# huawei-noah/Speech-Backbones

Measured on AMD Instinct MI355X. Metric: mel-frames/sec at N=50 reverse-diffusion, 80x1024 batch, higher is better.
Workload: dtype f32 storage, f16 hi*hi MFMA + fp8 cross-term MFMA (3x3 Block convolutions, Upsample; bf16x3 elsewhere), f32 accumulate; 1 GPU; BASELINE config 2: Grad-TTS LJSpeech decoder, N=50, B=16/GPU synthetic 80x1024 mels, all-ones mask; per_gpu_batch=16, frames=1024, parallelism=utterance-shard x1, weights=seed-0 default init, Rezero.g=0.02, output_finite=True, conv_kernel=conv_ws.hip (persistent, wave-specialised), sub_batch_streams=0, hip_graph=False, launches_per_euler_step=64

## Files before the change

speech-backbones_amd/csrc/attn.hip:

```cpp
#include <cstring>
#include "common.h"
#include "kernels.h"

#ifndef GTTS_ATTN_HPW
#define GTTS_ATTN_HPW 2
#endif

namespace gtts {

struct AttnCtxArgs {
    const void *x;
    const unsigned char *wkv;
    float *partials;
    int C, HW, nstage, tiles, tps, nrec, nsplit, B;
    AttnTail tail;
};

__device__ __forceinline__ void pack8_split(const float (&v)[8], u32x4 &hi, u32x4 &lo) {
    bf16x8 vh, vl;
#pragma unroll
    for (int i = 0; i < 8; ++i) {
        __bf16 h, l;
        split_bf16(v[i], h, l);
        vh[i] = h;
        vl[i] = l;
    }
    hi = *reinterpret_cast<u32x4 *>(&vh);
    lo = *reinterpret_cast<u32x4 *>(&vl);
}

template <int NSPLIT, int FULLC, typename AT = float, int HPW = 1, int TAIL = 0>
__global__ __launch_bounds__(256 * HPW, HPW == 1 ? 2 : 1) void attn_ctx_kernel(const AttnCtxArgs a) {
    constexpr int AB = (int)sizeof(AT);
    static_assert(!TAIL || (FULLC && AB == 4), "the fused tail: whole 32-channel stages, fp32 storage");
    constexpr int KCH = ATTN_KCH, NKG = 2 * KCH;
    constexpr int NKGT = NKG / HPW;
    constexpr int WHEAD = 2 * NKG * 64;
    static_assert(HPW == 1 || HPW == 2, "one or two heads per workgroup");
    constexpr int SM16 = 2 * NKG * 256 + HPW * WHEAD;
    static_assert((size_t)SM16 * 16 >= (size_t)4 * HPW * ATTN_REC * 4, "merge records must fit the staging buffer");
    __shared__ __attribute__((aligned(16))) u32x4 s_all[SM16];
    u32x4 *s_ah = s_all, *s_al = s_all + NKG * 256;
    u32x4 *s_wall = s_all + 2 * NKG * 256;

    const int tid = threadIdx.x, lane = tid & 63;
    const int t255 = tid & 255, hw = __builtin_amdgcn_readfirstlane(tid >> 8);
    const int wave = (tid >> 6) & 3;
    const int l31 = lane & 31, kgl = lane >> 5;
    constexpr int HG = 4 / HPW;
    const int nsl = gridDim.x / (HG * a.B);
    const int wg = xcd_slot(blockIdx.x, gridDim.x);
    const int head = (wg % HG) * HPW + hw, slice = (wg / HG) % nsl, b = (wg / HG) / nsl;
    u32x4 *s_w = s_wall + hw * WHEAD;
    const int tile0 = slice * a.tps;
    const int tile1 = min(tile0 + a.tps, a.tiles);
    const AT *xb = reinterpret_cast<const AT *>(a.x) + (size_t)b * a.C * a.HW;
    const u32x4 *wblk = reinterpret_cast<const u32x4 *>(a.wkv) + (size_t)head * a.nstage * (2 * NKG * 64);

    float raw[NKGT][8];
    u32x4 wregs[KCH];
    const unsigned long long xaddr = reinterpret_cast<unsigned long long>(xb);
    const unsigned xlo = __builtin_amdgcn_readfirstlane((unsigned)xaddr);
    const unsigned xhi = __builtin_amdgcn_readfirstlane((unsigned)(xaddr >> 32));
    const int xbytes = a.C * a.HW * AB;
    const __amdgpu_buffer_rsrc_t rsx = __builtin_amdgcn_make_buffer_rsrc(
        reinterpret_cast<void *>(((unsigned long long)xhi << 32) | xlo), 0, __builtin_amdgcn_readfirstlane(xbytes), 0x00020000);
    [[maybe_unused]] float rawh[NKGT][8], tmask = 0.f;
    [[maybe_unused]] __amdgpu_buffer_rsrc_t rsh = rsx, rsi = rsx;
    [[maybe_unused]] const bool tail_store = (wg % HG) == 0;
    if constexpr (TAIL) {
        auto mk = [&](const void *p) {
            const unsigned long long u = reinterpret_cast<unsigned long long>(reinterpret_cast<const AT *>(p) + (size_t)b * a.C * a.HW);
            const unsigned lo = __builtin_amdgcn_readfirstlane((unsigned)u), hi = __builtin_amdgcn_readfirstlane((unsigned)(u >> 32));
            return __builtin_amdgcn_make_buffer_rsrc(reinterpret_cast<void *>(((unsigned long long)hi << 32) | lo), 0,
                                                     __builtin_amdgcn_readfirstlane(xbytes), 0x00020000);
        };
        rsh = mk(a.tail.h);
        rsi = mk(a.tail.xin);
    }
    auto apply_tail = [&](int tile, int stage) {
        if constexpr (TAIL) {
            const int n = tile * 256 + t255;
            const int voff = n < a.HW ? n * AB : xbytes;
#pragma unroll
            for (int kg = 0; kg < NKGT; ++kg) {
                const int cb = stage * 16 * KCH + (hw * NKGT + kg) * 8;
#pragma unroll
                for (int i = 0; i < 8; ++i) {
                    const float sc = a.tail.esc[(size_t)b * a.C + cb + i], sh = a.tail.esh[(size_t)b * a.C + cb + i];
                    const float v = tail_value(rawh[kg][i], raw[kg][i], sc, sh, tmask);
                    raw[kg][i] = v;
                    if (tail_store) __builtin_amdgcn_raw_buffer_store_b32(__builtin_bit_cast(int, v), rsx, voff, (cb + i) * a.HW * 4, GTTS_OUT_NT);
                }
            }
        }
    };
    auto load = [&](int tile, int stage) {
        const int n = tile * 256 + t255;
        const int voff = n < a.HW ? n * AB : xbytes;
        if constexpr (TAIL) {
            if (stage == 0) tmask = n < a.HW ? a.tail.mask[(size_t)b * a.tail.T + ((size_t)(n % a.tail.W) << a.tail.lvl)] : 0.f;
        }
#pragma unroll
        for (int kg = 0; kg < NKGT; ++kg) {
            const int cb = stage * 16 * KCH + (hw * NKGT + kg) * 8;
#pragma unroll
            for (int i = 0; i < 8; ++i) {
                const int c = FULLC ? cb + i : min(cb + i, a.C - 1);
                float v;
                if constexpr (TAIL) {
                    v = __builtin_bit_cast(float, __builtin_amdgcn_raw_buffer_load_b32(rsi, voff, c * a.HW * 4, 0));
                    rawh[kg][i] = __builtin_bit_cast(float, __builtin_amdgcn_raw_buffer_load_b32(rsh, voff, c * a.HW * 4, 0));
                } else if constexpr (AB == 4) v = __builtin_bit_cast(float, __builtin_amdgcn_raw_buffer_load_b32(rsx, voff, c * a.HW * 4, 0));
                else v = __builtin_bit_cast(float, (unsigned)(unsigned short)__builtin_amdgcn_raw_buffer_load_b16(rsx, voff, c * a.HW * 2, 0) << 16);
                raw[kg][i] = (FULLC || cb + i < a.C) ? v : 0.f;
            }
        }
        const u32x4 *g = wblk + (size_t)stage * (2 * NKG * 64);
#pragma unroll
        for (int j = 0; j < KCH; ++j) wregs[j] = g[t255 + j * 256];
    };

    const float NEG_INF = -__builtin_inff();
    float m_run = NEG_INF, z_run = 0.f;
    f32x16 ctx;
#pragma unroll
    for (int r = 0; r < 16; ++r) ctx[r] = 0.f;
    constexpr bool lo_on = NSPLIT > 1;

    load(tile0, 0);
    for (int tile = tile0; tile < tile1; ++tile) {
        f32x16 acc[2][2];
#pragma unroll
        for (int pf = 0; pf < 2; ++pf)
#pragma unroll
            for (int cf = 0; cf < 2; ++cf)
#pragma unroll
                for (int r = 0; r < 16; ++r) acc[pf][cf][r] = 0.f;

        for (int stage = 0; stage < a.nstage; ++stage) {
            apply_tail(tile, stage);
            lds_barrier();
#pragma unroll
            for (int kg = 0; kg < NKGT; ++kg) {
                u32x4 hi, lo;
                pack8_split(raw[kg], hi, lo);
                s_ah[(hw * NKGT + kg) * 256 + t255] = hi;
                s_al[(hw * NKGT + kg) * 256 + t255] = lo;
            }
#pragma unroll
            for (int j = 0; j < KCH; ++j) s_w[t255 + j * 256] = wregs[j];
            lds_barrier();
            if (stage + 1 < a.nstage) load(tile, stage + 1);
            else if (tile + 1 < tile1) load(tile + 1, 0);
#pragma unroll
            for (int kc = 0; kc < KCH; ++kc) {
                bf16x8 xh[2], xl[2], wh[2], wl[2];
#pragma unroll
                for (int pf = 0; pf < 2; ++pf) {
                    const int xi = (kc * 2 + kgl) * 256 + wave * 64 + pf * 32 + l31;
                    xh[pf] = *reinterpret_cast<const bf16x8 *>(&s_ah[xi]);
                    xl[pf] = *reinterpret_cast<const bf16x8 *>(&s_al[xi]);
                }
#pragma unroll
                for (int cf = 0; cf < 2; ++cf) {
                    const int wi = (kc * 2 + kgl) * 64 + cf * 32 + l31;
                    wh[cf] = *reinterpret_cast<const bf16x8 *>(&s_w[wi]);
                    wl[cf] = *reinterpret_cast<const bf16x8 *>(&s_w[wi + NKG * 64]);
                }
#pragma unroll
                for (int pf = 0; pf < 2; ++pf)
#pragma unroll
                    for (int cf = 0; cf < 2; ++cf) {
                        if (lo_on) {
                            acc[pf][cf] = __builtin_amdgcn_mfma_f32_32x32x16_bf16(xl[pf], wh[cf], acc[pf][cf], 0, 0, 0);
                            acc[pf][cf] = __builtin_amdgcn_mfma_f32_32x32x16_bf16(xh[pf], wl[cf], acc[pf][cf], 0, 0, 0);
                        }
                        acc[pf][cf] = __builtin_amdgcn_mfma_f32_32x32x16_bf16(xh[pf], wh[cf], acc[pf][cf], 0, 0, 0);
                    }
            }
        }

        const int nbase = tile * 256 + wave * 64 + 4 * kgl;
        const bool full = tile * 256 + 256 <= a.HW;
        float tmax = NEG_INF;
        if (full) {
#pragma unroll
            for (int pf = 0; pf < 2; ++pf)
#pragma unroll
                for (int rg = 0; rg < 16; ++rg) tmax = fmaxf(tmax, acc[pf][0][rg]);
        } else {
#pragma unroll
            for (int pf = 0; pf < 2; ++pf)
#pragma unroll
                for (int rg = 0; rg < 16; ++rg) {
                    const int n = nbase + pf * 32 + (rg & 3) + 8 * (rg >> 2);
                    if (n < a.HW) tmax = fmaxf(tmax, acc[pf][0][rg]);
                }
        }
        tmax = fmaxf(tmax, __shfl_xor(tmax, 32, 64));
        const float m_new = fmaxf(m_run, tmax);
        const float alpha = (m_run == NEG_INF) ? 0.f : __expf(m_run - m_new);
        const float msub = (m_new == NEG_INF) ? 0.f : m_new;
        constexpr float LOG2E = 1.44269504088896340736f;
        float psum = 0.f;
        if (full) {
#pragma unroll
            for (int pf = 0; pf < 2; ++pf)
#pragma unroll
                for (int rg = 0; rg < 16; ++rg) {
                    const float p = __builtin_amdgcn_exp2f((acc[pf][0][rg] - msub) * LOG2E);
                    acc[pf][0][rg] = p;
                    psum += p;
                }
        } else {
#pragma unroll
            for (int pf = 0; pf < 2; ++pf)
#pragma unroll
                for (int rg = 0; rg < 16; ++rg) {
                    const int n = nbase + pf * 32 + (rg & 3) + 8 * (rg >> 2);
                    const float p = (n < a.HW) ? __builtin_amdgcn_exp2f((acc[pf][0][rg] - msub) * LOG2E) : 0.f;
                    acc[pf][0][rg] = p;
                    psum += p;
                }
        }
        psum += __shfl_xor(psum, 32, 64);
        z_run = z_run * alpha + psum;
        m_run = m_new;
        if (__builtin_amdgcn_ballot_w64(alpha != 1.f) != 0ull) {
#pragma unroll
            for (int rg = 0; rg < 16; ++rg) {
                const int d = (rg & 3) + 8 * (rg >> 2) + 4 * kgl;
                ctx[rg] *= __shfl(alpha, d, 64);
            }
        }
#pragma unroll
        for (int pf = 0; pf < 2; ++pf)
#pragma unroll
            for (int hh = 0; hh < 2; ++hh) {
                float pv[8], vv[8];
#pragma unroll
                for (int i = 0; i < 8; ++i) {
                    pv[i] = acc[pf][0][hh * 8 + i];
                    vv[i] = acc[pf][1][hh * 8 + i];
                }
                u32x4 ph, pl, vh, vl;
                pack8_split(pv, ph, pl);
                pack8_split(vv, vh, vl);
                const bf16x8 Ph = *reinterpret_cast<bf16x8 *>(&ph), Pl = *reinterpret_cast<bf16x8 *>(&pl);
                const bf16x8 Vh = *reinterpret_cast<bf16x8 *>(&vh), Vl = *reinterpret_cast<bf16x8 *>(&vl);
                if (lo_on) {
                    ctx = __builtin_amdgcn_mfma_f32_32x32x16_bf16(Pl, Vh, ctx, 0, 0, 0);
                    ctx = __builtin_amdgcn_mfma_f32_32x32x16_bf16(Ph, Vl, ctx, 0, 0, 0);
                }
                ctx = __builtin_amdgcn_mfma_f32_32x32x16_bf16(Ph, Vh, ctx, 0, 0, 0);
            }
    }

    __syncthreads();
    float (*s_mrg)[ATTN_REC] = reinterpret_cast<float (*)[ATTN_REC]>(s_all) + hw * 4;
    {
        float *mine = s_mrg[wave];
        if (kgl == 0) {
            mine[l31] = m_run;
            mine[32 + l31] = z_run;
        }
#pragma unroll
        for (int rg = 0; rg < 16; ++rg) {
            const int d = (rg & 3) + 8 * (rg >> 2) + 4 * kgl;
            mine[64 + d * 32 + l31] = ctx[rg];
        }
    }
    __syncthreads();
    float *rec = a.partials + ((((size_t)b * 4 + head) * a.nrec) + (size_t)slice) * ATTN_REC;
#pragma unroll
    for (int k = 0; k < 4; ++k) {
        const int idx = t255 + 256 * k, d = idx >> 5;
        float M = NEG_INF;
#pragma unroll
        for (int w = 0; w < 4; ++w) M = fmaxf(M, s_mrg[w][d]);
        float acc_c = 0.f, acc_z = 0.f;
#pragma unroll
        for (int w = 0; w < 4; ++w) {
            const float mw = s_mrg[w][d];
            const float sc = (mw == NEG_INF) ? 0.f : __expf(mw - M);
            acc_c = fmaf(s_mrg[w][64 + idx], sc, acc_c);
            acc_z = fmaf(s_mrg[w][32 + d], sc, acc_z);
        }
        rec[64 + idx] = acc_c;
        if ((idx & 31) == 0) {
            rec[d] = M;
            rec[32 + d] = acc_z;
        }
    }
}

template <int NSPLIT, typename AT, int TAIL = 0>
__global__ __launch_bounds__(256, 2) void attn_ctx64_kernel(const AttnCtxArgs a) {
    constexpr int AB = (int)sizeof(AT);
    constexpr int C = 64, NKGT = C / 8;
    constexpr bool lo_on = NSPLIT > 1;
    __shared__ __attribute__((aligned(16))) u32x4 s_ah[NKGT * 64];
    __shared__ __attribute__((aligned(16))) u32x4 s_al[NKGT * 64];
    __shared__ __attribute__((aligned(16))) u32x4 s_w[4][1024];

    const int tid = threadIdx.x, lane = tid & 63;
    const int wave = __builtin_amdgcn_readfirstlane(tid >> 6);
    const int l31 = lane & 31, kgl = lane >> 5;
    const int nsl = gridDim.x / a.B;
    const int wg = xcd_slot(blockIdx.x, gridDim.x);
    const int slice = wg % nsl, b = wg / nsl;
    const int head = wave;
    const int tile0 = slice * a.tps, tile1 = min(tile0 + a.tps, a.tiles);
    const AT *xb = reinterpret_cast<const AT *>(a.x) + (size_t)b * C * a.HW;

    {
        const u32x4 *wsrc = reinterpret_cast<const u32x4 *>(a.wkv) + (size_t)head * 1024;
        u32x4 wr[16];
#pragma unroll
        for (int i = 0; i < 16; ++i) wr[i] = wsrc[lane + 64 * i];
#pragma unroll
        for (int i = 0; i < 16; ++i) s_w[wave][lane + 64 * i] = wr[i];
    }

    const unsigned long long xaddr = reinterpret_cast<unsigned long long>(xb);
    const unsigned xlo = __builtin_amdgcn_readfirstlane((unsigned)xaddr);
    const unsigned xhi = __builtin_amdgcn_readfirstlane((unsigned)(xaddr >> 32));
    const int xbytes = C * a.HW * AB;
    const __amdgpu_buffer_rsrc_t rsx = __builtin_amdgcn_make_buffer_rsrc(
        reinterpret_cast<void *>(((unsigned long long)xhi << 32) | xlo), 0, __builtin_amdgcn_readfirstlane(xbytes), 0x00020000);
    float raw[2][8];
    [[maybe_unused]] float rawh[2][8], tsc[2][8], tsh[2][8], tmask = 0.f;
    [[maybe_unused]] __amdgpu_buffer_rsrc_t rsh = rsx, rsi = rsx;
    if constexpr (TAIL) {
        static_assert(!TAIL || AB == 4, "the fused tail is the fp32-storage form");
        auto mk = [&](const void *p) {
            const unsigned long long u = reinterpret_cast<unsigned long long>(reinterpret_cast<const AT *>(p) + (size_t)b * C * a.HW);
            const unsigned lo = __builtin_amdgcn_readfirstlane((unsigned)u), hi = __builtin_amdgcn_readfirstlane((unsigned)(u >> 32));
            return __builtin_amdgcn_make_buffer_rsrc(reinterpret_cast<void *>(((unsigned long long)hi << 32) | lo), 0,
                                                     __builtin_amdgcn_readfirstlane(xbytes), 0x00020000);
        };
        rsh = mk(a.tail.h);
        rsi = mk(a.tail.xin);
#pragma unroll
        for (int it = 0; it < 2; ++it)
#pragma unroll
            for (int i = 0; i < 8; ++i) {
                const int c = (it * 4 + wave) * 8 + i;
                tsc[it][i] = a.tail.esc[(size_t)b * C + c];
                tsh[it][i] = a.tail.esh[(size_t)b * C + c];
            }
    }
    auto load = [&](int tile) {
        const int n = tile * 64 + lane;
        const int voff = n < a.HW ? n * AB : xbytes;
#pragma unroll
        for (int it = 0; it < 2; ++it)
#pragma unroll
            for (int i = 0; i < 8; ++i) {
                const int c = (it * 4 + wave) * 8 + i;
                if constexpr (TAIL) {
                    raw[it][i] = __builtin_bit_cast(float, __builtin_amdgcn_raw_buffer_load_b32(rsi, voff, c * a.HW * 4, 0));
                    rawh[it][i] = __builtin_bit_cast(float, __builtin_amdgcn_raw_buffer_load_b32(rsh, voff, c * a.HW * 4, 0));
                } else if constexpr (AB == 4) raw[it][i] = __builtin_bit_cast(float, __builtin_amdgcn_raw_buffer_load_b32(rsx, voff, c * a.HW * 4, 0));
                else raw[it][i] = __builtin_bit_cast(float, (unsigned)(unsigned short)__builtin_amdgcn_raw_buffer_load_b16(rsx, voff, c * a.HW * 2, 0) << 16);
            }
        if constexpr (TAIL) tmask = n < a.HW ? a.tail.mask[(size_t)b * a.tail.T + ((size_t)(n % a.tail.W) << a.tail.lvl)] : 0.f;
    };
    auto apply_tail = [&](int tile) {
        if constexpr (TAIL) {
            const int n = tile * 64 + lane;
            const int voff = n < a.HW ? n * AB : xbytes;
#pragma unroll
            for (int it = 0; it < 2; ++it)
#pragma unroll
                for (int i = 0; i < 8; ++i) {
                    const int c = (it * 4 + wave) * 8 + i;
                    const float v = tail_value(rawh[it][i], raw[it][i], tsc[it][i], tsh[it][i], tmask);
                    raw[it][i] = v;
                    __builtin_amdgcn_raw_buffer_store_b32(__builtin_bit_cast(int, v), rsx, voff, c * a.HW * 4, GTTS_OUT_NT);
                }
        }
    };

    const float NEG_INF = -__builtin_inff();
    float m_run = NEG_INF, z_run = 0.f;
    f32x16 ctx;
#pragma unroll
    for (int r = 0; r < 16; ++r) ctx[r] = 0.f;

    load(tile0);
    for (int tile = tile0; tile < tile1; ++tile) {
        apply_tail(tile);
        lds_barrier();
#pragma unroll
        for (int it = 0; it < 2; ++it) {
            u32x4 hi, lo;
            pack8_split(raw[it], hi, lo);
            s_ah[(it * 4 + wave) * 64 + lane] = hi;
            if (lo_on) s_al[(it * 4 + wave) * 64 + lane] = lo;
        }
        lds_barrier();
        load(min(tile + 1, tile1 - 1));

        f32x16 acc[2][2];
#pragma unroll
        for (int pf = 0; pf < 2; ++pf)
#pragma unroll
            for (int cf = 0; cf < 2; ++cf)
#pragma unroll
                for (int r = 0; r < 16; ++r) acc[pf][cf][r] = 0.f;
#pragma unroll
        for (int s = 0; s < 4; ++s) {
            bf16x8 xh[2], xl[2], wh[2], wl[2];
#pragma unroll
            for (int pf = 0; pf < 2; ++pf) {
                const int xi = (s * 2 + kgl) * 64 + pf * 32 + l31;
                xh[pf] = *reinterpret_cast<const bf16x8 *>(&s_ah[xi]);
                if (lo_on) xl[pf] = *reinterpret_cast<const bf16x8 *>(&s_al[xi]);
            }
#pragma unroll
            for (int cf = 0; cf < 2; ++cf) {
                const int wi = (s >> 1) * 512 + ((s & 1) * 2 + kgl) * 64 + cf * 32 + l31;
                wh[cf] = *reinterpret_cast<const bf16x8 *>(&s_w[wave][wi]);
                if (lo_on) wl[cf] = *reinterpret_cast<const bf16x8 *>(&s_w[wave][wi + 256]);
            }
#pragma unroll
            for (int pf = 0; pf < 2; ++pf)
#pragma unroll
                for (int cf = 0; cf < 2; ++cf) {
                    if (lo_on) {
                        acc[pf][cf] = __builtin_amdgcn_mfma_f32_32x32x16_bf16(xl[pf], wh[cf], acc[pf][cf], 0, 0, 0);
                        acc[pf][cf] = __builtin_amdgcn_mfma_f32_32x32x16_bf16(xh[pf], wl[cf], acc[pf][cf], 0, 0, 0);
                    }
                    acc[pf][cf] = __builtin_amdgcn_mfma_f32_32x32x16_bf16(xh[pf], wh[cf], acc[pf][cf], 0, 0, 0);
                }
        }

        const int nbase = tile * 64 + 4 * kgl;
        const bool full = tile * 64 + 64 <= a.HW;
        float tmax = NEG_INF;
        if (full) {
#pragma unroll
            for (int pf = 0; pf < 2; ++pf)
#pragma unroll
                for (int rg = 0; rg < 16; ++rg) tmax = fmaxf(tmax, acc[pf][0][rg]);
        } else {
#pragma unroll
            for (int pf = 0; pf < 2; ++pf)
#pragma unroll
                for (int rg = 0; rg < 16; ++rg) {
                    const int n = nbase + pf * 32 + (rg & 3) + 8 * (rg >> 2);
                    if (n < a.HW) tmax = fmaxf(tmax, acc[pf][0][rg]);
                }
        }
        tmax = fmaxf(tmax, __shfl_xor(tmax, 32, 64));
        const float m_new = fmaxf(m_run, tmax);
        const float alpha = (m_run == NEG_INF) ? 0.f : __expf(m_run - m_new);
        const float msub = (m_new == NEG_INF) ? 0.f : m_new;
        constexpr float LOG2E = 1.44269504088896340736f;
        float psum = 0.f;
        if (full) {
#pragma unroll
            for (int pf = 0; pf < 2; ++pf)
#pragma unroll
                for (int rg = 0; rg < 16; ++rg) {
                    const float p = __builtin_amdgcn_exp2f((acc[pf][0][rg] - msub) * LOG2E);
                    acc[pf][0][rg] = p;
                    psum += p;
                }
        } else {
#pragma unroll
            for (int pf = 0; pf < 2; ++pf)
#pragma unroll
                for (int rg = 0; rg < 16; ++rg) {
                    const int n = nbase + pf * 32 + (rg & 3) + 8 * (rg >> 2);
                    const float p = (n < a.HW) ? __builtin_amdgcn_exp2f((acc[pf][0][rg] - msub) * LOG2E) : 0.f;
                    acc[pf][0][rg] = p;
                    psum += p;
                }
        }
        psum += __shfl_xor(psum, 32, 64);
        z_run = z_run * alpha + psum;
        m_run = m_new;
        if (__builtin_amdgcn_ballot_w64(alpha != 1.f) != 0ull) {
#pragma unroll
            for (int rg = 0; rg < 16; ++rg) {
                const int d = (rg & 3) + 8 * (rg >> 2) + 4 * kgl;
                ctx[rg] *= __shfl(alpha, d, 64);
            }
        }
#pragma unroll
        for (int pf = 0; pf < 2; ++pf)
#pragma unroll
            for (int hh = 0; hh < 2; ++hh) {
                float pv[8], vv[8];
#pragma unroll
                for (int i = 0; i < 8; ++i) {
                    pv[i] = acc[pf][0][hh * 8 + i];
                    vv[i] = acc[pf][1][hh * 8 + i];
                }
                u32x4 ph, pl, vh, vl;
                pack8_split(pv, ph, pl);
                pack8_split(vv, vh, vl);
                const bf16x8 Ph = *reinterpret_cast<bf16x8 *>(&ph), Pl = *reinterpret_cast<bf16x8 *>(&pl);
                const bf16x8 Vh = *reinterpret_cast<bf16x8 *>(&vh), Vl = *reinterpret_cast<bf16x8 *>(&vl);
                if (lo_on) {
                    ctx = __builtin_amdgcn_mfma_f32_32x32x16_bf16(Pl, Vh, ctx, 0, 0, 0);
                    ctx = __builtin_amdgcn_mfma_f32_32x32x16_bf16(Ph, Vl, ctx, 0, 0, 0);
                }
                ctx = __builtin_amdgcn_mfma_f32_32x32x16_bf16(Ph, Vh, ctx, 0, 0, 0);
            }
    }

    float *rec = a.partials + ((((size_t)b * 4 + head) * a.nrec) + (size_t)slice) * ATTN_REC;
    if (kgl == 0) {
        rec[l31] = m_run;
        rec[32 + l31] = z_run;
    }
#pragma unroll
    for (int rg = 0; rg < 16; ++rg) {
        const int d = (rg & 3) + 8 * (rg >> 2) + 4 * kgl;
        rec[64 + d * 32 + l31] = ctx[rg];
    }
}

template <int NSPLIT, typename AT, int TAIL>
static hipError_t launch_ctx64(const AttnCtxArgs &a, dim3 grid, hipStream_t st, std::string *name) {
    if (name) return kernel_name(name, "gtts::attn_ctx64_kernel", NSPLIT, act_name<AT>(), TAIL);
    hipLaunchKernelGGL((attn_ctx64_kernel<NSPLIT, AT, TAIL>), grid, dim3(256), 0, st, a);
    return hipGetLastError();
}
template <int NSPLIT, int FULLC, typename AT, int TAIL>
static hipError_t launch_ctx(const AttnCtxArgs &a, int nslices, hipStream_t st, std::string *name) {
    constexpr int HPW = GTTS_ATTN_HPW;
    if (name) return kernel_name(name, "gtts::attn_ctx_kernel", NSPLIT, FULLC, act_name<AT>(), HPW, TAIL);
    hipLaunchKernelGGL((attn_ctx_kernel<NSPLIT, FULLC, AT, HPW, TAIL>), dim3(nslices * (4 / HPW) * a.B), dim3(256 * HPW), 0, st, a);
    return hipGetLastError();
}

hipError_t launch_attn_ctx(const void *x, const unsigned char *wkv, float *partials, int B, int C, int HW, int nsplit,
                           hipStream_t st, int act_bf16, const AttnTail *tail, std::string *name) {
    AttnGeom g = attn_geom(HW, C);
    if ((size_t)C * HW * 4 >= ((size_t)1 << 31)) return hipErrorInvalidValue;
    if (tail != nullptr && (C % 32 != 0 || act_bf16)) return hipErrorInvalidValue;
    if (act_bf16 && nsplit > 1) return hipErrorInvalidValue;
    AttnCtxArgs a;
    memset(&a, 0, sizeof(a));
    if (tail != nullptr) a.tail = *tail;
    a.x = x; a.wkv = wkv; a.partials = partials; a.C = C; a.HW = HW;
    a.nstage = (C + 16 * ATTN_KCH - 1) / (16 * ATTN_KCH);
    a.tiles = g.tiles; a.tps = g.tps; a.nrec = g.nrec; a.nsplit = nsplit; a.B = B;
    if (attn_head_per_wave(C)) {
        static_assert(ATTN_KCH == 2, "attn_ctx64_kernel indexes the packed k|v blocks as 32-channel stages");
        const dim3 grid64(g.nslices * B);
        if (act_bf16) return launch_ctx64<1, __bf16, 0>(a, grid64, st, name);
        if (tail != nullptr) return nsplit > 1 ? launch_ctx64<2, float, 1>(a, grid64, st, name) : launch_ctx64<1, float, 1>(a, grid64, st, name);
        return nsplit > 1 ? launch_ctx64<2, float, 0>(a, grid64, st, name) : launch_ctx64<1, float, 0>(a, grid64, st, name);
    }
    if (act_bf16) return C % 32 == 0 ? launch_ctx<1, 1, __bf16, 0>(a, g.nslices, st, name) : launch_ctx<1, 0, __bf16, 0>(a, g.nslices, st, name);
    if (tail != nullptr) return nsplit > 1 ? launch_ctx<2, 1, float, 1>(a, g.nslices, st, name) : launch_ctx<1, 1, float, 1>(a, g.nslices, st, name);
    if (C % 32 == 0) return nsplit > 1 ? launch_ctx<2, 1, float, 0>(a, g.nslices, st, name) : launch_ctx<1, 1, float, 0>(a, g.nslices, st, name);
    return nsplit > 1 ? launch_ctx<2, 0, float, 0>(a, g.nslices, st, name) : launch_ctx<1, 0, float, 0>(a, g.nslices, st, name);
}

__global__ __launch_bounds__(1024) void attn_merge_kernel(const float *__restrict__ partials, float *__restrict__ ctxn,
                                                           int nrec) {
    extern __shared__ float sm[];
    float *s_w = sm;
    float *s_red = sm + (size_t)nrec * 32;
    float *s_M = s_red + 1024;
    float *s_Zi = s_M + 32;
    const int head = blockIdx.x, b = blockIdx.y, tid = threadIdx.x;
    const int d = tid & 31, g = tid >> 5;
    const float *rec = partials + ((size_t)b * 4 + head) * nrec * ATTN_REC;
    const float NEG_INF = -__builtin_inff();
    float mx = NEG_INF;
    for (int i = g; i < nrec; i += 32) mx = fmaxf(mx, rec[(size_t)i * ATTN_REC + d]);
    s_red[g * 32 + d] = mx;
    __syncthreads();
    if (g == 0) {
        float M = NEG_INF;
        for (int k = 0; k < 32; ++k) M = fmaxf(M, s_red[k * 32 + d]);
        s_M[d] = M;
    }
    __syncthreads();
    const float M = s_M[d];
    float zz = 0.f;
    for (int i = g; i < nrec; i += 32) {
        const float mi = rec[(size_t)i * ATTN_REC + d];
        const float w = (mi == NEG_INF) ? 0.f : expf(mi - M);
        s_w[i * 32 + d] = w;
        zz += rec[(size_t)i * ATTN_REC + 32 + d] * w;
    }
    __syncthreads();
    s_red[g * 32 + d] = zz;
    __syncthreads();
    if (g == 0) {
        float Z = 0.f;
        for (int k = 0; k < 32; ++k) Z += s_red[k * 32 + d];
        s_Zi[d] = 1.0f / Z;
    }
    __syncthreads();
    const int dd = tid >> 5;
    float acc = 0.f;
    const float *cp = rec + 64 + tid;
    int i = 0;
    for (; i + 4 <= nrec; i += 4) {
        const float c0 = cp[(size_t)(i + 0) * ATTN_REC], c1 = cp[(size_t)(i + 1) * ATTN_REC];
        const float c2 = cp[(size_t)(i + 2) * ATTN_REC], c3 = cp[(size_t)(i + 3) * ATTN_REC];
        acc = fmaf(c0, s_w[(i + 0) * 32 + dd], acc);
        acc = fmaf(c1, s_w[(i + 1) * 32 + dd], acc);
        acc = fmaf(c2, s_w[(i + 2) * 32 + dd], acc);
        acc = fmaf(c3, s_w[(i + 3) * 32 + dd], acc);
    }
    for (; i < nrec; ++i) acc = fmaf(cp[(size_t)i * ATTN_REC], s_w[i * 32 + dd], acc);
    ctxn[(((size_t)b * 4 + head) * 1024) + tid] = acc * s_Zi[dd];
}

hipError_t launch_attn_merge(const float *partials, float *ctxn, int B, int nrec, hipStream_t st) {
    const size_t smem = ((size_t)nrec * 32 + 1024 + 64) * sizeof(float);
    if (smem > 160 * 1024) return hipErrorInvalidValue;
    if (smem > 48 * 1024) {
        const hipError_t e = raise_dyn_lds<&attn_merge_kernel>(smem);
        if (e != hipSuccess) return e;
    }
    hipLaunchKernelGGL(attn_merge_kernel, dim3(4, B), dim3(1024), smem, st, partials, ctxn, nrec);
    return hipGetLastError();
}

constexpr int FOLD_CO = 8;
struct AttnFoldArgs {
    const float *ctxn, *wq, *wout, *bout, *g;
    unsigned char *wpk;
    size_t wpk_bstride;
    float *biasb;
    int C, MT, nkg;
    int ndn;
    const float *dn_w, *dn_wo, *dn_vw;
    unsigned char *dn_wpk;
    size_t dn_bstride;
    float *dn_btab;
    int dn_MT, dn_nkg;
};
__global__ __launch_bounds__(256) void attn_fold_kernel(const AttnFoldArgs a) {
    __shared__ float s_U[FOLD_CO][128];
    __shared__ float s_part[4][FOLD_CO][128];
    const int co0 = blockIdx.x * FOLD_CO, b = blockIdx.z, tid = threadIdx.x;
    const int C = a.C;
    const int tap = (int)blockIdx.y < a.ndn ? (int)blockIdx.y : -1;
    const float *wout = tap >= 0 ? a.dn_wo + (size_t)tap * C * 128 : a.wout;
    const float *cb = a.ctxn + (size_t)b * 4096;
    {
        const int j = tid & 127, h = j >> 5, d = j & 31;
        const float4 *cx = reinterpret_cast<const float4 *>(cb + (h * 32 + d) * 32);
        float4 cv[8];
#pragma unroll
        for (int e = 0; e < 8; ++e) cv[e] = cx[e];
#pragma unroll
        for (int rr = 0; rr < FOLD_CO / 2; ++rr) {
            const int r = (tid >> 7) * (FOLD_CO / 2) + rr;
            const float4 *wo = reinterpret_cast<const float4 *>(wout + (size_t)(co0 + r) * 128 + h * 32);
            float acc = 0.f;
#pragma unroll
            for (int e = 0; e < 8; ++e) {
                const float4 w4 = wo[e];
                acc = fmaf(w4.x, cv[e].x, acc); acc = fmaf(w4.y, cv[e].y, acc);
                acc = fmaf(w4.z, cv[e].z, acc); acc = fmaf(w4.w, cv[e].w, acc);
            }
            s_U[r][j] = acc;
        }
    }
    __syncthreads();
    const float gv = a.g[0];
    const int MT = tap >= 0 ? a.dn_MT : a.MT, nkg = tap >= 0 ? a.dn_nkg : a.nkg;
    const int ncot = (C + MT - 1) / MT;
    __bf16 *wp = tap >= 0 ? reinterpret_cast<__bf16 *>(a.dn_wpk + (size_t)b * a.dn_bstride)
                          : reinterpret_cast<__bf16 *>(a.wpk + (size_t)b * a.wpk_bstride);
    const int ky = tap >= 0 ? tap / 3 : 0, kx = tap >= 0 ? tap - 3 * ky : 0;
    const int nst = tap >= 0 ? 3 : 1, tps = nst;
    const int Cc = C < 256 ? C : 256;
    const int nj = 256 / Cc >= 4 ? 4 : (256 / Cc >= 2 ? 2 : 1);
    const int jq = tid / Cc, cl = tid - jq * Cc;
    const int jn = 128 / nj;
    const bool active = jq < nj;
    for (int ci = cl; ci < C; ci += Cc) {
        float acc[FOLD_CO];
#pragma unroll
        for (int r = 0; r < FOLD_CO; ++r) acc[r] = 0.f;
        const float *qp = a.wq + (size_t)(active ? jq * jn : 0) * C + ci;
        for (int j0 = 0; j0 < (active ? jn : 0); j0 += 8) {
            float q[8];
#pragma unroll
            for (int u = 0; u < 8; ++u) q[u] = qp[(size_t)(j0 + u) * C];
#pragma unroll
            for (int u = 0; u < 8; ++u)
#pragma unroll
                for (int r = 0; r < FOLD_CO; ++r) acc[r] = fmaf(s_U[r][jq * jn + j0 + u], q[u], acc[r]);
        }
        if (nj > 1) {
            if (active && jq > 0) {
#pragma unroll
                for (int r = 0; r < FOLD_CO; ++r) s_part[jq][r][cl] = acc[r];
            }
            __syncthreads();
            if (jq == 0) {
                for (int k = 1; k < nj; ++k)
#pragma unroll
                    for (int r = 0; r < FOLD_CO; ++r) acc[r] += s_part[k][r][cl];
            }
        }
        if (jq == 0) {
            const int chunk = ci / (8 * nkg), kg = (ci >> 3) % nkg, i = ci & 7;
#pragma unroll
            for (int r = 0; r < FOLD_CO; ++r) {
                const int co = co0 + r, cot = co / MT, m = co % MT;
                const size_t blk = ((size_t)chunk * nst + ky) * ncot + cot;
                const size_t blk_elems = (size_t)tps * MT * 16 * nkg;
                const size_t e_hi = blk * blk_elems + ((size_t)((0 * tps + kx) * nkg + kg) * MT + m) * 8 + i;
                const size_t e_lo = blk * blk_elems + ((size_t)((1 * tps + kx) * nkg + kg) * MT + m) * 8 + i;
                const float v = tap >= 0 ? fmaf(acc[r], gv, a.dn_w[((size_t)co * C + ci) * 9 + tap]) : acc[r] * gv;
                __bf16 hi, lo;
                split_bf16(v, hi, lo);
                wp[e_hi] = hi;
                wp[e_lo] = lo;
            }
        }
    }
    if (tap < 0 && tid < FOLD_CO) a.biasb[(size_t)b * C + co0 + tid] = gv * a.bout[co0 + tid];
    if (tap == 0 && tid < FOLD_CO) {
        const int co = co0 + tid;
        float *t = a.dn_btab + (size_t)b * 6 * C + co;
#pragma unroll
        for (int k = 0; k < 3; ++k) {
            const float v0 = a.dn_vw[(size_t)(0 + k) * C + co], v1 = a.dn_vw[(size_t)(3 + k) * C + co], v2 = a.dn_vw[(size_t)(6 + k) * C + co];
            t[(size_t)(0 + k) * C] = gv * (v1 + v2);
            t[(size_t)(3 + k) * C] = gv * ((v0 + v1) + v2);
        }
    }
}

hipError_t launch_attn_fold(const float *ctxn, const float *wq, const float *wout, const float *bout, const float *g,
                            unsigned char *wpk, size_t wpk_bstride, float *biasb, int B, int C, hipStream_t st,
                            const AttnFoldDn *dn) {
    if (C % 16 != 0) return hipErrorInvalidValue;
    ConvGeom geom = conv_geom(CONV_P1, C, C);
    if (C % (16 * geom.kch) != 0) return hipErrorInvalidValue;
    if (wpk == nullptr && dn == nullptr) return hipErrorInvalidValue;
    AttnFoldArgs a;
    memset(&a, 0, sizeof(a));
    a.ctxn = ctxn; a.wq = wq; a.wout = wout; a.bout = bout; a.g = g;
    a.wpk = wpk; a.wpk_bstride = wpk_bstride; a.biasb = biasb;
    a.C = C; a.MT = geom.MT; a.nkg = 2 * geom.kch;
    if (dn != nullptr) {
        ConvGeom gd = conv_geom(CONV_DN, C, C);
        if (C % (16 * gd.kch) != 0 || C % gd.MT != 0 || gd.nst != 3 || gd.tps != 3) return hipErrorInvalidValue;
        if (dn->bstride < conv_packed_bytes(CONV_DN, C, C)) return hipErrorInvalidValue;
        a.ndn = 9;
        a.dn_w = dn->w; a.dn_wo = dn->wo; a.dn_vw = dn->vw;
        a.dn_wpk = dn->wpk; a.dn_bstride = dn->bstride; a.dn_btab = dn->btab;
        a.dn_MT = gd.MT; a.dn_nkg = 2 * gd.kch;
    }
    hipLaunchKernelGGL(attn_fold_kernel, dim3(C / FOLD_CO, a.ndn + (wpk != nullptr ? 1 : 0), B), dim3(256), 0, st, a);
    return hipGetLastError();
}

__global__ __launch_bounds__(128) void attn_dn_precompose_kernel(const float *__restrict__ w, const float *__restrict__ wout,
                                                                  const float *__restrict__ bout, float *__restrict__ wo,
                                                                  float *__restrict__ vw, int C) {
    const int co = blockIdx.x, tap = blockIdx.y, j = threadIdx.x;
    const float *wr = w + (size_t)co * C * 9 + tap;
    float acc = 0.f, accb = 0.f;
    for (int c = 0; c < C; ++c) {
        const float wv = wr[(size_t)c * 9];
        acc = fmaf(wv, wout[(size_t)c * 128 + j], acc);
        accb = fmaf(wv, bout[c], accb);
    }
    wo[((size_t)tap * C + co) * 128 + j] = acc;
    if (j == 0) vw[(size_t)tap * C + co] = accb;
}

hipError_t launch_attn_dn_precompose(const float *w, const float *wout, const float *bout, float *wo, float *vw, int C, hipStream_t st) {
    hipLaunchKernelGGL(attn_dn_precompose_kernel, dim3(C, 9), dim3(128), 0, st, w, wout, bout, wo, vw, C);
    return hipGetLastError();
}

}
```

Before: 55910 mel-frames/s.

## Split attention merge across row groups and vectorize fold weight packing stores

The merge kernel now splits each head across four smaller workgroups when there are many partial records, and hoists the first two record loads into registers to cut load latency. The fold kernel is templated on the j-split factor. It prefetches q weights through buffer loads with double buffering and reads s_U as float4. It stages packed bf16 hi/lo weights in LDS so they can be written as 16-byte vector stores instead of scattered 2-byte stores. Optional memtime tracing instrumentation is added behind a debug macro, and new alignment checks reject unaligned packed-weight buffers.

```diff
diff --git a/speech-backbones_amd/csrc/attn.hip b/speech-backbones_amd/csrc/attn.hip
--- a/speech-backbones_amd/csrc/attn.hip
+++ b/speech-backbones_amd/csrc/attn.hip
@@ -564,68 +564,134 @@
     return nsplit > 1 ? launch_ctx<2, 0, float, 0>(a, g.nslices, st, name) : launch_ctx<1, 0, float, 0>(a, g.nslices, st, name);
 }
 
+#ifndef GTTS_DIAG
+#undef GTTS_GLUE_TRACE
+#endif
+#ifndef GTTS_GLUE_TRACE
+#define GTTS_GLUE_TRACE 0
+#endif
+#if GTTS_GLUE_TRACE
+constexpr int GLUE_TRACE_MERGE = 4, GLUE_TRACE_N = 8 * 16 * 16 * 9;
+__device__ unsigned long long g_glue_trace[GLUE_TRACE_N];
+extern "C" int gtts_debug_trace_glue(unsigned long long *dst, int n) {
+    return (int)hipMemcpyFromSymbol(dst, HIP_SYMBOL(g_glue_trace), sizeof(unsigned long long) * (n < GLUE_TRACE_N ? n : GLUE_TRACE_N));
+}
+__device__ __forceinline__ int merge_trace_slot(int nrec) { return nrec == 16 ? 0 : (nrec == 20 ? 1 : (nrec == 64 ? 2 : 3)); }
+__device__ __forceinline__ unsigned long long *glue_trace_row(int slot, int wg, int wave) {
+    return g_glue_trace + (((size_t)slot * 16 + wg) * 16 + wave) * 9;
+}
+#define MT_MARK(k) do { const unsigned long long tr_now = __builtin_amdgcn_s_memtime(); tr_sum[k] += tr_now - tr_t; tr_t = tr_now; } while (0)
+#else
+#define MT_MARK(k) do { } while (0)
+#endif
 __global__ __launch_bounds__(1024) void attn_merge_kernel(const float *__restrict__ partials, float *__restrict__ ctxn,
                                                            int nrec) {
     extern __shared__ float sm[];
+    const int RD = (int)blockDim.x >> 5;
+    const int R = 32 / RD;
     float *s_w = sm;
-    float *s_red = sm + (size_t)nrec * 32;
-    float *s_M = s_red + 1024;
-    float *s_Zi = s_M + 32;
-    const int head = blockIdx.x, b = blockIdx.y, tid = threadIdx.x;
-    const int d = tid & 31, g = tid >> 5;
+    float *s_red = sm + (size_t)nrec * RD;
+    float *s_M = s_red + 32 * RD;
+    float *s_Zi = s_M + RD;
+    const int head = (int)blockIdx.x / R, row0 = ((int)blockIdx.x - head * R) * RD, b = blockIdx.y, tid = threadIdx.x;
+    const int d = tid & (RD - 1), g = tid / RD;
+#if GTTS_GLUE_TRACE
+    const bool tr_on = (tid & 63) == 0;
+    unsigned long long tr_sum[8] = {0, 0, 0, 0, 0, 0, 0, 0};
+    unsigned long long tr_t = __builtin_amdgcn_s_memtime();
+    const unsigned long long tr_entry = tr_t;
+#endif
     const float *rec = partials + ((size_t)b * 4 + head) * nrec * ATTN_REC;
+    const float *recd = rec + row0 + d;
     const float NEG_INF = -__builtin_inff();
-    float mx = NEG_INF;
-    for (int i = g; i < nrec; i += 32) mx = fmaxf(mx, rec[(size_t)i * ATTN_REC + d]);
-    s_red[g * 32 + d] = mx;
+    const bool h0 = g < nrec, h1 = g + 32 < nrec;
+    const float *r0 = recd + (size_t)(h0 ? g : 0) * ATTN_REC, *r1 = recd + (size_t)(h1 ? g + 32 : 0) * ATTN_REC;
+    const float m0 = r0[0], m1 = r1[0], z0 = r0[32], z1 = r1[32];
+    float mx = fmaxf(h0 ? m0 : NEG_INF, h1 ? m1 : NEG_INF);
+    for (int i = g + 64; i < nrec; i += 32) mx = fmaxf(mx, recd[(size_t)i * ATTN_REC]);
+    MT_MARK(0);
+    s_red[g * RD + d] = mx;
     __syncthreads();
     if (g == 0) {
         float M = NEG_INF;
-        for (int k = 0; k < 32; ++k) M = fmaxf(M, s_red[k * 32 + d]);
+        for (int k = 0; k < 32; ++k) M = fmaxf(M, s_red[k * RD + d]);
         s_M[d] = M;
     }
     __syncthreads();
+    MT_MARK(1);
     const float M = s_M[d];
     float zz = 0.f;
-    for (int i = g; i < nrec; i += 32) {
-        const float mi = rec[(size_t)i * ATTN_REC + d];
+    if (h0) {
+        const float w = (m0 == NEG_INF) ? 0.f : expf(m0 - M);
+        s_w[g * RD + d] = w;
+        zz += z0 * w;
+    }
+    if (h1) {
+        const float w = (m1 == NEG_INF) ? 0.f : expf(m1 - M);
+        s_w[(g + 32) * RD + d] = w;
+        zz += z1 * w;
+    }
+    for (int i = g + 64; i < nrec; i += 32) {
+        const float mi = recd[(size_t)i * ATTN_REC];
         const float w = (mi == NEG_INF) ? 0.f : expf(mi - M);
-        s_w[i * 32 + d] = w;
-        zz += rec[(size_t)i * ATTN_REC + 32 + d] * w;
+        s_w[i * RD + d] = w;
+        zz += recd[(size_t)i * ATTN_REC + 32] * w;
     }
     __syncthreads();
-    s_red[g * 32 + d] = zz;
+    s_red[g * RD + d] = zz;
     __syncthreads();
     if (g == 0) {
         float Z = 0.f;
-        for (int k = 0; k < 32; ++k) Z += s_red[k * 32 + d];
+        for (int k = 0; k < 32; ++k) Z += s_red[k * RD + d];
         s_Zi[d] = 1.0f / Z;
     }
     __syncthreads();
+    MT_MARK(2);
     const int dd = tid >> 5;
     float acc = 0.f;
-    const float *cp = rec + 64 + tid;
+    const float *cp = rec + 64 + row0 * 32 + tid;
     int i = 0;
+    for (; i + 16 <= nrec; i += 16) {
+        float c[16];
+#pragma unroll
+        for (int u = 0; u < 16; ++u) c[u] = cp[(size_t)(i + u) * ATTN_REC];
+#pragma unroll
+        for (int u = 0; u < 16; ++u) acc = fmaf(c[u], s_w[(i + u) * RD + dd], acc);
+    }
     for (; i + 4 <= nrec; i += 4) {
         const float c0 = cp[(size_t)(i + 0) * ATTN_REC], c1 = cp[(size_t)(i + 1) * ATTN_REC];
         const float c2 = cp[(size_t)(i + 2) * ATTN_REC], c3 = cp[(size_t)(i + 3) * ATTN_REC];
-        acc = fmaf(c0, s_w[(i + 0) * 32 + dd], acc);
-        acc = fmaf(c1, s_w[(i + 1) * 32 + dd], acc);
-        acc = fmaf(c2, s_w[(i + 2) * 32 + dd], acc);
-        acc = fmaf(c3, s_w[(i + 3) * 32 + dd], acc);
-    }
-    for (; i < nrec; ++i) acc = fmaf(cp[(size_t)i * ATTN_REC], s_w[i * 32 + dd], acc);
-    ctxn[(((size_t)b * 4 + head) * 1024) + tid] = acc * s_Zi[dd];
-}
+        acc = fmaf(c0, s_w[(i + 0) * RD + dd], acc);
+        acc = fmaf(c1, s_w[(i + 1) * RD + dd], acc);
+        acc = fmaf(c2, s_w[(i + 2) * RD + dd], acc);
+        acc = fmaf(c3, s_w[(i + 3) * RD + dd], acc);
+    }
+    for (; i < nrec; ++i) acc = fmaf(cp[(size_t)i * ATTN_REC], s_w[i * RD + dd], acc);
+    MT_MARK(3);
+    ctxn[(((size_t)b * 4 + head) * 1024) + row0 * 32 + tid] = acc * s_Zi[dd];
+#if GTTS_GLUE_TRACE
+    if (tr_on && blockIdx.y == 0 && blockIdx.x < 16) {
+        __builtin_amdgcn_s_waitcnt(0);
+        MT_MARK(4);
+        unsigned long long *t = glue_trace_row(GLUE_TRACE_MERGE + merge_trace_slot(nrec), blockIdx.x, tid >> 6);
+        for (int q = 0; q < 8; ++q) t[q] = tr_sum[q];
+        t[8] = tr_t - tr_entry;
+    }
+#endif
+}
+
+static inline int attn_merge_row_groups(int nrec) { return nrec >= 48 ? 4 : 1; }
 
 hipError_t launch_attn_merge(const float *partials, float *ctxn, int B, int nrec, hipStream_t st) {
-    const size_t smem = ((size_t)nrec * 32 + 1024 + 64) * sizeof(float);
+    if (nrec < 1) return hipErrorInvalidValue;
+    const int R = attn_merge_row_groups(nrec);
+    const size_t smem = ((size_t)nrec * (32 / R) + 1024 / R + 2 * (32 / R)) * sizeof(float);
     if (smem > 160 * 1024) return hipErrorInvalidValue;
     if (smem > 48 * 1024) {
         const hipError_t e = raise_dyn_lds<&attn_merge_kernel>(smem);
         if (e != hipSuccess) return e;
     }
-    hipLaunchKernelGGL(attn_merge_kernel, dim3(4, B), dim3(1024), smem, st, partials, ctxn, nrec);
+    hipLaunchKernelGGL(attn_merge_kernel, dim3(4 * R, B), dim3(1024 / R), smem, st, partials, ctxn, nrec);
     return hipGetLastError();
 }
 
@@ -643,14 +709,58 @@
     float *dn_btab;
     int dn_MT, dn_nkg;
 };
-__global__ __launch_bounds__(256) void attn_fold_kernel(const AttnFoldArgs a) {
-    __shared__ float s_U[FOLD_CO][128];
-    __shared__ float s_part[4][FOLD_CO][128];
+constexpr int FOLD_QB = 32;
+template <int NJ>
+__device__ __forceinline__ void attn_fold_impl(const AttnFoldArgs &a, float (*s_U)[128], float (*s_part)[FOLD_CO][128],
+                                               __bf16 (*s_o)[FOLD_CO][256 + 8]) {
+    constexpr int JN = 128 / NJ;
+    constexpr int QB = FOLD_QB;
+    constexpr int NB = JN / QB;
     const int co0 = blockIdx.x * FOLD_CO, b = blockIdx.z, tid = threadIdx.x;
     const int C = a.C;
     const int tap = (int)blockIdx.y < a.ndn ? (int)blockIdx.y : -1;
     const float *wout = tap >= 0 ? a.dn_wo + (size_t)tap * C * 128 : a.wout;
     const float *cb = a.ctxn + (size_t)b * 4096;
+    const int Cc = C < 256 ? C : 256;
+    const int jq = tid / Cc, cl = tid - jq * Cc;
+    const bool active = jq < NJ;
+    const int jb = (active ? jq : 0) * JN;
+#if GTTS_GLUE_TRACE
+    const bool tr_on = (tid & 63) == 0;
+    unsigned long long tr_sum[8] = {0, 0, 0, 0, 0, 0, 0, 0};
+    unsigned long long tr_t = __builtin_amdgcn_s_memtime();
+    const unsigned long long tr_entry = tr_t;
+#endif
+    float q[2][QB], dw[FOLD_CO];
+#pragma unroll
+    for (int r = 0; r < FOLD_CO; ++r) dw[r] = 0.f;
+    int ci0 = 0, cis = cl;
+    auto rsrc = [](const float *p, int bytes) {
+        const unsigned long long u = reinterpret_cast<unsigned long long>(p);
+        const unsigned lo = __builtin_amdgcn_readfirstlane((unsigned)u), hi = __builtin_amdgcn_readfirstlane((unsigned)(u >> 32));
+        return __builtin_amdgcn_make_buffer_rsrc(reinterpret_cast<void *>(((unsigned long long)hi << 32) | lo), 0,
+                                                 __builtin_amdgcn_readfirstlane(bytes), 0x00020000);
+    };
+    const __amdgpu_buffer_rsrc_t rs_q = rsrc(a.wq, 128 * C * 4);
+    const __amdgpu_buffer_rsrc_t rs_w = rsrc(tap >= 0 ? a.dn_w : a.wq, tap >= 0 ? C * C * 36 : 128 * C * 4);
+    auto load_q = [&](float (&dst)[QB], int kb) {
+        const int voff = (jb * C + cis) * 4;
+#pragma unroll
+        for (int u = 0; u < QB; ++u)
+            dst[u] = __builtin_bit_cast(float, __builtin_amdgcn_raw_buffer_load_b32(rs_q, voff, (kb * QB + u) * C * 4, 0));
+    };
+    auto preload = [&]() {
+        load_q(q[0], 0);
+        if (NB > 1) load_q(q[1], 1);
+        if (tap >= 0 && jq == 0) {
+#pragma unroll
+            for (int r = 0; r < FOLD_CO; ++r)
+                dw[r] = __builtin_bit_cast(float, __builtin_amdgcn_raw_buffer_load_b32(rs_w, cis * 36, ((co0 + r) * C * 9 + tap) * 4, 0));
+        }
+    };
+    const float gv = a.g[0];
+    preload();
+    MT_MARK(0);
     {
         const int j = tid & 127, h = j >> 5, d = j & 31;
         const float4 *cx = reinterpret_cast<const float4 *>(cb + (h * 32 + d) * 32);
@@ -671,61 +781,77 @@
             s_U[r][j] = acc;
         }
     }
+    MT_MARK(1);
     __syncthreads();
-    const float gv = a.g[0];
+    MT_MARK(2);
     const int MT = tap >= 0 ? a.dn_MT : a.MT, nkg = tap >= 0 ? a.dn_nkg : a.nkg;
     const int ncot = (C + MT - 1) / MT;
     __bf16 *wp = tap >= 0 ? reinterpret_cast<__bf16 *>(a.dn_wpk + (size_t)b * a.dn_bstride)
                           : reinterpret_cast<__bf16 *>(a.wpk + (size_t)b * a.wpk_bstride);
     const int ky = tap >= 0 ? tap / 3 : 0, kx = tap >= 0 ? tap - 3 * ky : 0;
     const int nst = tap >= 0 ? 3 : 1, tps = nst;
-    const int Cc = C < 256 ? C : 256;
-    const int nj = 256 / Cc >= 4 ? 4 : (256 / Cc >= 2 ? 2 : 1);
-    const int jq = tid / Cc, cl = tid - jq * Cc;
-    const int jn = 128 / nj;
-    const bool active = jq < nj;
-    for (int ci = cl; ci < C; ci += Cc) {
+    const size_t blk_elems = (size_t)tps * MT * 16 * nkg;
+    const int ngrp = Cc >> 3;
+    for (;;) {
         float acc[FOLD_CO];
 #pragma unroll
         for (int r = 0; r < FOLD_CO; ++r) acc[r] = 0.f;
-        const float *qp = a.wq + (size_t)(active ? jq * jn : 0) * C + ci;
-        for (int j0 = 0; j0 < (active ? jn : 0); j0 += 8) {
-            float q[8];
-#pragma unroll
-            for (int u = 0; u < 8; ++u) q[u] = qp[(size_t)(j0 + u) * C];
-#pragma unroll
-            for (int u = 0; u < 8; ++u)
-#pragma unroll
-                for (int r = 0; r < FOLD_CO; ++r) acc[r] = fmaf(s_U[r][jq * jn + j0 + u], q[u], acc[r]);
-        }
-        if (nj > 1) {
+#pragma unroll
+        for (int kb = 0; kb < NB; ++kb) {
+#pragma unroll
+            for (int j0 = 0; j0 < QB; j0 += 4) {
+#pragma unroll
+                for (int r = 0; r < FOLD_CO; ++r) {
+                    const float4 u4 = *reinterpret_cast<const float4 *>(&s_U[r][jb + kb * QB + j0]);
+                    acc[r] = fmaf(u4.x, q[kb & 1][j0 + 0], acc[r]);
+                    acc[r] = fmaf(u4.y, q[kb & 1][j0 + 1], acc[r]);
+                    acc[r] = fmaf(u4.z, q[kb & 1][j0 + 2], acc[r]);
+                    acc[r] = fmaf(u4.w, q[kb & 1][j0 + 3], acc[r]);
+                }
+            }
+            if (kb + 2 < NB) load_q(q[kb & 1], kb + 2);
+        }
+        if (NJ > 1) {
             if (active && jq > 0) {
 #pragma unroll
-                for (int r = 0; r < FOLD_CO; ++r) s_part[jq][r][cl] = acc[r];
+                for (int r = 0; r < FOLD_CO; ++r) s_part[jq - 1][r][cl] = acc[r];
             }
             __syncthreads();
             if (jq == 0) {
-                for (int k = 1; k < nj; ++k)
-#pragma unroll
-                    for (int r = 0; r < FOLD_CO; ++r) acc[r] += s_part[k][r][cl];
+                for (int k = 1; k < NJ; ++k)
+#pragma unroll
+                    for (int r = 0; r < FOLD_CO; ++r) acc[r] += s_part[k - 1][r][cl];
             }
         }
         if (jq == 0) {
-            const int chunk = ci / (8 * nkg), kg = (ci >> 3) % nkg, i = ci & 7;
 #pragma unroll
             for (int r = 0; r < FOLD_CO; ++r) {
+                const float v = tap >= 0 ? fmaf(acc[r], gv, dw[r]) : acc[r] * gv;
+                __bf16 hi, lo;
+                split_bf16(v, hi, lo);
+                s_o[0][r][cl] = hi;
+                s_o[1][r][cl] = lo;
+            }
+        }
+        __syncthreads();
+        MT_MARK(5);
+        for (int un = tid; un < 2 * FOLD_CO * ngrp; un += 256) {
+            const int r = un & (FOLD_CO - 1), gh = un / FOLD_CO, grp = gh % ngrp, half = gh / ngrp;
+            const int ci = ci0 + grp * 8;
+            if (ci < C) {
+                const int chunk = ci / (8 * nkg), kg = (ci >> 3) % nkg;
                 const int co = co0 + r, cot = co / MT, m = co % MT;
                 const size_t blk = ((size_t)chunk * nst + ky) * ncot + cot;
-                const size_t blk_elems = (size_t)tps * MT * 16 * nkg;
-                const size_t e_hi = blk * blk_elems + ((size_t)((0 * tps + kx) * nkg + kg) * MT + m) * 8 + i;
-                const size_t e_lo = blk * blk_elems + ((size_t)((1 * tps + kx) * nkg + kg) * MT + m) * 8 + i;
-                const float v = tap >= 0 ? fmaf(acc[r], gv, a.dn_w[((size_t)co * C + ci) * 9 + tap]) : acc[r] * gv;
-                __bf16 hi, lo;
-                split_bf16(v, hi, lo);
-                wp[e_hi] = hi;
-                wp[e_lo] = lo;
-            }
-        }
+                const size_t e = blk * blk_elems + ((size_t)((half * tps + kx) * nkg + kg) * MT + m) * 8;
+                *reinterpret_cast<uint4 *>(wp + e) = *reinterpret_cast<const uint4 *>(&s_o[half][r][grp * 8]);
+            }
+        }
+        MT_MARK(6);
+        ci0 += Cc;
+        if (ci0 >= C) break;
+        __syncthreads();
+        cis = ci0 + cl < C ? ci0 + cl : cl;
+        preload();
     }
     if (tap < 0 && tid < FOLD_CO) a.biasb[(size_t)b * C + co0 + tid] = gv * a.bout[co0 + tid];
     if (tap == 0 && tid < FOLD_CO) {
@@ -738,6 +864,25 @@
             t[(size_t)(3 + k) * C] = gv * ((v0 + v1) + v2);
         }
     }
+#if GTTS_GLUE_TRACE
+    if (tr_on && blockIdx.z == 0 && blockIdx.x < 16 && (tap == 0 || tap < 0)) {
+        __builtin_amdgcn_s_waitcnt(0);
+        MT_MARK(7);
+        unsigned long long *t = glue_trace_row(C == 64 ? (tap >= 0 ? 0 : 1) : (C == 128 ? 2 : 3), blockIdx.x, tid >> 6);
+        for (int k = 0; k < 8; ++k) t[k] = tr_sum[k];
+        t[8] = tr_t - tr_entry;
+    }
+#endif
+}
+
+__global__ __launch_bounds__(256) __attribute__((amdgpu_waves_per_eu(2))) void attn_fold_kernel(const AttnFoldArgs a) {
+    __shared__ __attribute__((aligned(16))) float s_U[FOLD_CO][128];
+    __shared__ float s_part[3][FOLD_CO][128];
+    __shared__ __attribute__((aligned(16))) __bf16 s_o[2][FOLD_CO][256 + 8];
+    const int nj = a.C <= 64 ? 4 : (a.C <= 128 ? 2 : 1);
+    if (nj == 4) attn_fold_impl<4>(a, s_U, s_part, s_o);
+    else if (nj == 2) attn_fold_impl<2>(a, s_U, s_part, s_o);
+    else attn_fold_impl<1>(a, s_U, s_part, s_o);
 }
 
 hipError_t launch_attn_fold(const float *ctxn, const float *wq, const float *wout, const float *bout, const float *g,
@@ -747,6 +892,8 @@
     ConvGeom geom = conv_geom(CONV_P1, C, C);
     if (C % (16 * geom.kch) != 0) return hipErrorInvalidValue;
     if (wpk == nullptr && dn == nullptr) return hipErrorInvalidValue;
+    if ((uintptr_t)wpk % 16 != 0 || wpk_bstride % 16 != 0) return hipErrorInvalidValue;
+    if (dn != nullptr && ((uintptr_t)dn->wpk % 16 != 0 || dn->bstride % 16 != 0)) return hipErrorInvalidValue;
     AttnFoldArgs a;
     memset(&a, 0, sizeof(a));
     a.ctxn = ctxn; a.wq = wq; a.wout = wout; a.bout = bout; a.g = g;
```

Result: no change. 55880 mel-frames/s (-0.1%).
